# Yzmblog/SurfD

Measured on AMD Instinct MI355X. Metric: shapes/sec end-to-end (1000-step uncond, 512^3 UDF) at 1/2/4/8 GPU, higher is better.
Workload: dtype f32 (every matrix product of decoder and denoiser as three split-fp16 products on the fp16 MFMA pipe with fp32 accumulation — fp32-class error, same golden tolerances as the exact-fp32 kernels; samplers, attention, embedding MLP and grid bookkeeping in exact fp32)

## Files before the change

### surfd_amd/csrc/decoder.hip

```cpp
#include "common.h"
#include "points.h"
#include <string.h>
#include <stdlib.h>
#include <type_traits>
#include <utility>

namespace surfd {

constexpr int H = 512;
constexpr int NB = 5;
constexpr int NCBN = 2 * NB + 1;
constexpr int TP = 64;
constexpr int XS = H + 4;
constexpr int ES = 68;
constexpr int KG_H = H / 8;
constexpr int KG_E = 8;

constexpr size_t SZ_FCP = (size_t)16 * KG_E * 256;
constexpr size_t SZ_HH = (size_t)16 * KG_H * 256;
constexpr size_t SZ_FCPT = (size_t)2 * KG_H * 256;
constexpr size_t OFF_FCP = 0;
__host__ __device__ constexpr size_t off_fc(int k, int which) { return SZ_FCP + (size_t)(2 * k + which) * SZ_HH; }
__host__ __device__ constexpr size_t off_fcT(int k, int which) { return SZ_FCP + (size_t)(2 * NB + 2 * k + which) * SZ_HH; }
constexpr size_t OFF_FCPT = SZ_FCP + (size_t)4 * NB * SZ_HH;
// ... 218 lines not shown
#pragma unroll
    for (int d = REQ_EARLY ? REQ_EARLY_UPTO : WS_AHEAD; d < D - 1; ++d) load_wstage<KS>(ws.b[d], Whf, lofs, d);
#pragma unroll 1
    for (int ks0 = 0; ks0 < KS - D; ks0 += D) group(ks0, std::false_type{});
    group(KS - D, std::true_type{});
}

template <int... I, typename F>
__device__ __forceinline__ void static_for_impl(std::integer_sequence<int, I...>, F &&f) { (f(std::integral_constant<int, I>{}), ...); }
template <int N, typename F>
__device__ __forceinline__ void static_for(F &&f) { static_for_impl(std::make_integer_sequence<int, N>{}, f); }

template <int BEG, bool WITH_CHUNKS, typename ChunkFn>
__device__ __forceinline__ void gemm_half_f16x2(const float *A, const _Float16 *Whf, WStages &ws, f32x16 (&acc)[2][4], int lane, ChunkFn &&chunk) {
    constexpr int D = 4, KS = KS_H, END = BEG + 16;
    const float *a0 = A + (lane & 31) * XS + 4 * (lane >> 5);
    const float *a1 = a0 + 32 * XS;
    unsigned lofs = (unsigned)lane * 16u;
    asm volatile("" : "+v"(lofs));
    f16x8 x[2][2][2];
    auto load_x = [&](f16x8 (&dst)[2][2], int ks) {
        dst[0][0] = *reinterpret_cast<const f16x8 *>(a0 + ks * 8); dst[0][1] = *reinterpret_cast<const f16x8 *>(a0 + 256 + ks * 8);
        dst[1][0] = *reinterpret_cast<const f16x8 *>(a1 + ks * 8); dst[1][1] = *reinterpret_cast<const f16x8 *>(a1 + 256 + ks * 8);
    };
    load_x(x[0], BEG);
    if constexpr (BEG == 0) {
#pragma unroll
        for (int d = REQ_EARLY ? REQ_EARLY_UPTO : 0; d < D - 1; ++d) load_wstage<KS>(ws.b[d], Whf, lofs, d);
    }
    if constexpr (WITH_CHUNKS) {
        static_for<16>([&](auto idx) {
            constexpr int ks = BEG + decltype(idx)::value, j = ks % D;
            if constexpr (ks + D - 1 < KS) load_wstage<KS>(ws.b[(j + D - 1) % D], Whf, lofs, ks + D - 1);
            if constexpr (ks + 1 < END) load_x(x[(ks + 1) & 1], ks + 1);
            chunk(idx);
            mfma_step_f16x2(x[ks & 1], ws.b[j], acc);
#pragma unroll
            for (int i = 0; i < 8; ++i) { __builtin_amdgcn_sched_group_barrier(0x008, 1, 0); __builtin_amdgcn_sched_group_barrier(0x020, 1, 0); __builtin_amdgcn_sched_group_barrier(0x002, 1, 0); }
#pragma unroll
            for (int i = 0; i < 4; ++i) { __builtin_amdgcn_sched_group_barrier(0x008, 1, 0); __builtin_amdgcn_sched_group_barrier(0x100, 1, 0); __builtin_amdgcn_sched_group_barrier(0x002, 2, 0); }
#pragma unroll
            for (int i = 0; i < 8; ++i) { __builtin_amdgcn_sched_group_barrier(0x008, 1, 0); __builtin_amdgcn_sched_group_barrier(0x002, 2, 0); }
#pragma unroll
            for (int i = 0; i < 4; ++i) { __builtin_amdgcn_sched_group_barrier(0x008, 1, 0); __builtin_amdgcn_sched_group_barrier(0x200, 1, 0); }
            __builtin_amdgcn_sched_barrier(0);
        });
    } else {
        auto group = [&](int ks0, auto last) {
            int goff = ks0 * 8;
            asm volatile("" : "+v"(goff));
#pragma unroll
            for (int j = 0; j < D; ++j) {
                if (!decltype(last)::value || j == 0) load_wstage<KS>(ws.b[(j + D - 1) % D], Whf, lofs, ks0 + j + D - 1);
                const int jn = (decltype(last)::value && j == D - 1) ? j : j + 1;
                x[(j + 1) & 1][0][0] = *reinterpret_cast<const f16x8 *>(a0 + goff + jn * 8); x[(j + 1) & 1][0][1] = *reinterpret_cast<const f16x8 *>(a0 + goff + 256 + jn * 8);
                x[(j + 1) & 1][1][0] = *reinterpret_cast<const f16x8 *>(a1 + goff + jn * 8); x[(j + 1) & 1][1][1] = *reinterpret_cast<const f16x8 *>(a1 + goff + 256 + jn * 8);
                mfma_step_f16x2(x[j & 1], ws.b[j], acc);
#pragma unroll
                for (int i = 0; i < 8; ++i) { __builtin_amdgcn_sched_group_barrier(0x008, 1, 0); __builtin_amdgcn_sched_group_barrier(0x020, 1, 0); }
#pragma unroll
                for (int i = 0; i < 4; ++i) { __builtin_amdgcn_sched_group_barrier(0x008, 1, 0); __builtin_amdgcn_sched_group_barrier(0x100, 1, 0); }
                __builtin_amdgcn_sched_group_barrier(0x008, 12, 0);
                __builtin_amdgcn_sched_barrier(0);
            }
        };
        static_assert(END == KS, "the rolled half is the second one");
#pragma unroll 1
        for (int ks0 = BEG; ks0 < END - D; ks0 += D) group(ks0, std::false_type{});
        group(END - D, std::true_type{});
    }
}

template <int KG>
__device__ __forceinline__ void gemm_1x1(const float *A, int astride, int mt, const gfloat *Wp_tile, f32x16 &acc, int lane) {
    const float *a0 = A + (32 * mt + (lane & 31)) * astride + 4 * (lane >> 5);
    const gf32x4 *w = reinterpret_cast<const gf32x4 *>(Wp_tile) + lane;
#pragma unroll 4
    for (int kg = 0; kg < KG; ++kg) {
        const f32x4 x0 = *reinterpret_cast<const f32x4 *>(a0 + kg * 8);
        const f32x4 b = w[kg * 64];
#pragma unroll
        for (int q = 0; q < 4; ++q) acc = mfma(x0[q], b[q], acc);
    }
}

__device__ __forceinline__ void zero_acc(f32x16 (&acc)[2][4]) {
#pragma unroll
    for (int mt = 0; mt < 2; ++mt)
#pragma unroll
        for (int nt = 0; nt < 4; ++nt)
#pragma unroll
            for (int r = 0; r < 16; ++r) acc[mt][nt][r] = 0.f;
}

__device__ __forceinline__ constexpr int mword(int mt, int nt) { return (mt * 4 + nt) >> 1; }
__device__ __forceinline__ constexpr int mbit(int mt, int nt, int r) { return ((mt * 4 + nt) & 1) * 16 + r; }

template <int TPP>
__device__ __forceinline__ void encode_tile_f16x2(const PtIO &io, long e0, long npts, const float *PT, float *X, int tid, int &sat_flag) {
    constexpr int LOG2 = TPP == 8 ? 3 : 2;
    static_assert(TPP == 4 || TPP == 8, "threads per point");
    const int p = tid >> LOG2, part = tid & (TPP - 1);
    _Float16 *hrow = reinterpret_cast<_Float16 *>(reinterpret_cast<unsigned *>(X) + p * XS);
    auto put = [&](int j, float u) {
        const _Float16 h = (_Float16)u;
        hrow[j] = h;
        hrow[512 + j] = (_Float16)(u - (float)h);
    };
    if (io.mode == PT_EMB) {
        const long e = e0 + p;
        bool bad = false;
#pragma unroll 2
        for (int i = 0; i < 64 / TPP; ++i) {
            const int j = part * (64 / TPP) + i;
            float u = (e < npts && j < io.emb_dim) ? io.xyz[e * io.emb_dim + j] : 0.f;
            bad |= __builtin_fabsf(u) > 65504.f;
            u = __builtin_amdgcn_fmed3f(u, -65504.f, 65504.f);
            put(j, u);
        }
        sat_flag |= __any(bad);
        return;
    }
    const float x = PT[p * 4 + 0], y = PT[p * 4 + 1], z = PT[p * 4 + 2];
    {
        float u = part == 0 ? x : (part == 1 ? y : z);
        const bool bad = part < 3 && __builtin_fabsf(u) > 65504.f;
        sat_flag |= __any(bad);
        u = __builtin_amdgcn_fmed3f(u, -65504.f, 65504.f);
        if (part < 3) put(part, u);
        if (part == 3) put(63, 0.f);
    }
    int f = part / 3, r = part - 3 * (part / 3);
#pragma unroll
    for (int q0 = 0; q0 < 30; q0 += TPP) {
        if (q0 + part < 30) {
            const float a = (r == 0 ? x : (r == 1 ? y : z)) * (float)(1 << f);
            float sn, cs;
            sincosf(a, &sn, &cs);
            put(3 + 6 * f + r, sn);
            put(6 + 6 * f + r, cs);
        }
        r += TPP % 3; f += TPP / 3;
        if (r >= 3) { r -= 3; ++f; }
    }
}

#ifdef SURFD_DEC_STAMPS
__device__ long long g_dec_stamps[8];
#define TDECL() long long tacc_[5] = {0, 0, 0, 0, 0}, t0_ = __builtin_readcyclecounter()
#define TADD(slot) do { const long long t1_ = __builtin_readcyclecounter(); tacc_[slot] += t1_ - t0_; t0_ = t1_; } while (0)
#define TBAR() do { TADD(tphase_); __syncthreads(); TADD(3); } while (0)
#define TPHASE(x) tphase_ = (x)
#define TFLUSH() do { if (blockIdx.x == 0 && threadIdx.x == 0) { for (int i_ = 0; i_ < 5; ++i_) g_dec_stamps[i_] += tacc_[i_]; g_dec_stamps[5] += 1; } } while (0)
#else
#define TDECL()
#define TADD(slot)
#define TBAR() __syncthreads()
#define TPHASE(x)
#define TFLUSH()
#endif

template <bool GRAD, bool F16X2 = false>
__global__ __launch_bounds__(256, 1) void decoder_kernel(DecParams P, PtBatch B) {
    extern __shared__ __attribute__((aligned(16))) float lds[];
    float *X = lds;
    float *E = lds;
    float *PT = lds + TP * XS;
    float *LOG = PT + TP * 4;
    float *E2 = LOG + TP;
    float *DV = E2 + TP * ES;
    float *RED = DV + TP * 4;

    const int tid = threadIdx.x, lane = tid & 63, wave = tid >> 6;
    const int col = lane & 31;
    const int wave_u = __builtin_amdgcn_readfirstlane(wave);
    typedef float __attribute__((address_space(3))) lds_f32;
    lds_f32 *xb0 = (lds_f32 *)(X + (4 * (lane >> 5)) * XS + 128 * wave + col);
    lds_f32 *xb1 = xb0 + 32 * XS;
    auto fresh_xat_bases = [&]() { if constexpr (GRAD && F16X2) asm volatile("" : "+v"(xb0), "+v"(xb1)); };
#define XAT(mt, nt, r) ((mt) ? xb1 : xb0)[(((r) & 3) + 8 * ((r) >> 2)) * XS + 32 * (nt)]
    typedef unsigned __attribute__((address_space(3))) lds_u32;
    lds_u32 *xw0 = (lds_u32 *)(reinterpret_cast<unsigned *>(X) + (4 * (lane >> 5)) * XS + XW_WAVE * wave + col);
    lds_u32 *xw1 = xw0 + 32 * XS;
#define XW(mt, q, r, pl) ((mt) ? xw1 : xw0)[(((r) & 3) + 8 * ((r) >> 2)) * XS + XW_Q * (q) + 256 * (pl)]
    int sat_flag = 0;
    auto store_split = [&](const f32x16 (&v)[2][4], const float (&sa)[4], const float (&sb)[4], unsigned *mk, auto qn) {
        float umax = 0.f;
#pragma unroll
        for (int q = 0; q < decltype(qn)::value; ++q)
#pragma unroll
            for (int mt = 0; mt < 2; ++mt) {
                if constexpr (!GRAD && !FWD_STAGED) {
#pragma unroll
                    for (int r = 0; r < 16; ++r) {
                        const float t0 = __builtin_fmaf(sa[2 * q], v[mt][2 * q][r], sb[2 * q]);
                        const float t1 = __builtin_fmaf(sa[2 * q + 1], v[mt][2 * q + 1][r], sb[2 * q + 1]);
                        umax = __builtin_fmaxf(__builtin_fmaxf(umax, t0), t1);
                        const float u0 = __builtin_amdgcn_fmed3f(t0, 0.f, 65504.f);
                        const float u1 = __builtin_amdgcn_fmed3f(t1, 0.f, 65504.f);
                        const f32x2 u = {u0, u1};
                        const unsigned h = __builtin_bit_cast(unsigned, __builtin_convertvector(u, f16x2));
                        XW(mt, q, r, 0) = h;
                        XW(mt, q, r, 1) = split_low_pair(h, u0, u1);
                    }
                    continue;
                }
                __builtin_amdgcn_sched_barrier(0);
#pragma unroll
                for (int r0 = 0; r0 < 16; r0 += SURFD_DEC_GRAD_W) {
                    float t0[SURFD_DEC_GRAD_W], t1[SURFD_DEC_GRAD_W];
                    f32x2 u[SURFD_DEC_GRAD_W];
                    f16x2 h[SURFD_DEC_GRAD_W];
                    unsigned l[SURFD_DEC_GRAD_W];
#pragma unroll
                    for (int i = 0; i < SURFD_DEC_GRAD_W; ++i) {
                        t0[i] = __builtin_fmaf(sa[2 * q], v[mt][2 * q][r0 + i], sb[2 * q]);
                        t1[i] = __builtin_fmaf(sa[2 * q + 1], v[mt][2 * q + 1][r0 + i], sb[2 * q + 1]);
                    }
#pragma unroll
                    for (int i = 0; i < SURFD_DEC_GRAD_W; ++i) {
                        umax = __builtin_fmaxf(__builtin_fmaxf(umax, t0[i]), t1[i]);
                        if constexpr (GRAD) {
                            mk[mword(mt, 2 * q)] |= t0[i] > 0.f ? 1u << mbit(mt, 2 * q, r0 + i) : 0u;
                            mk[mword(mt, 2 * q + 1)] |= t1[i] > 0.f ? 1u << mbit(mt, 2 * q + 1, r0 + i) : 0u;
                        }
                        u[i].x = __builtin_amdgcn_fmed3f(t0[i], 0.f, 65504.f);
                        u[i].y = __builtin_amdgcn_fmed3f(t1[i], 0.f, 65504.f);
                    }
#pragma unroll
                    for (int i = 0; i < SURFD_DEC_GRAD_W; ++i) h[i] = __builtin_convertvector(u[i], f16x2);
#pragma unroll
                    for (int i = 0; i < SURFD_DEC_GRAD_W; ++i) {
#if SURFD_DEC_GRAD_MIX
                        l[i] = split_low_pair(__builtin_bit_cast(unsigned, h[i]), u[i].x, u[i].y);
#else
                        l[i] = __builtin_bit_cast(unsigned, __builtin_convertvector(u[i] - __builtin_convertvector(h[i], f32x2), f16x2));
#endif
                    }
#pragma unroll
                    for (int i = 0; i < SURFD_DEC_GRAD_W; ++i) {
                        XW(mt, q, r0 + i, 0) = __builtin_bit_cast(unsigned, h[i]);
                        XW(mt, q, r0 + i, 1) = l[i];
                    }
                }
            }
        sat_flag |= __any(umax > 65504.f);
    };
    auto split_chunk = [&](auto idx, const f32x16 (&v)[2][4], const float (&sa)[4], const float (&sb)[4], float &umax) {
#pragma unroll
        for (int i = 0; i < 2; ++i) {
            constexpr int base = 2 * decltype(idx)::value;
            const int mt = (base + i) >> 4, r = (base + i) & 15;
            const float t0 = __builtin_fmaf(sa[2], v[mt][2][r], sb[2]);
            const float t1 = __builtin_fmaf(sa[3], v[mt][3][r], sb[3]);
            umax = __builtin_fmaxf(__builtin_fmaxf(umax, t0), t1);
            const float u0 = __builtin_amdgcn_fmed3f(t0, 0.f, 65504.f);
            const float u1 = __builtin_amdgcn_fmed3f(t1, 0.f, 65504.f);
            const f32x2 u = {u0, u1};
            const f16x2 h = __builtin_convertvector(u, f16x2);
            const f32x2 hf = __builtin_convertvector(h, f32x2);
            const f32x2 rr = {u0 - hf.x, u1 - hf.y};
            const f16x2 l = __builtin_convertvector(rr, f16x2);
            XW(mt, 1, r, 0) = __builtin_bit_cast(unsigned, h);
            XW(mt, 1, r, 1) = __builtin_bit_cast(unsigned, l);
        }
    };

    WStages ws;
    if constexpr (F16X2) gemm_prefetch_f16x2<KS_E>(ws, P.whf + (size_t)(4 * wave_u) * KS_E * 2 * 512, lane);

    TDECL(); int tphase_ = 0; (void)tphase_;
    for (int bi = 0; bi < B.n; ++bi) {
    const PtIO &io = B.io[bi];
    const long npts = pt_count(io);
    const long ntiles = (npts + TP - 1) / TP;
    const float *tab_sample = P.tab + (size_t)B.sample[bi] * NCBN * 2 * H;
    const long tstep = io.shard_n > 1 ? io.shard_n : 1;
    for (long tile = blockIdx.x * tstep + (io.shard_n > 1 ? io.shard_i : 0); tile < ntiles; tile += gridDim.x * tstep) {
        const long e0 = tile * TP;
        const float *wpack_ = P.wpack, *vecs_ = P.vecs, *tab_ = tab_sample;
        const _Float16 *whf = P.whf;
        int tid_tile = threadIdx.x;
        if constexpr (GRAD && F16X2) asm volatile("" : "+v"(tid_tile));
        const int tid = tid_tile, lane = tid & 63, wave = tid >> 6, col = lane & 31;
        int cb = 128 * wave + col;
        asm volatile("" : "+s"(wpack_), "+s"(vecs_), "+s"(tab_));
        if constexpr (F16X2) asm volatile("" : "+s"(whf), "+v"(cb), "+v"(xw0), "+v"(xw1));
        const gfloat *wpack = (const gfloat *)wpack_, *vecs = (const gfloat *)vecs_, *tab = (const gfloat *)tab_;
        TPHASE(4);
        TBAR();
        if (tid < TP) {
            const long e = e0 + tid;
            float x = 0.f, y = 0.f, z = 0.f;
            int vox = -1;
            if (e < npts) {
                if (io.mode == PT_XYZ) {
                    x = io.xyz[e * 3 + 0]; y = io.xyz[e * 3 + 1]; z = io.xyz[e * 3 + 2];
                    vox = 0;
                } else if (io.mode == PT_EMB) {
                    vox = 0;
                } else {
                    vox = pt_voxel(io, e);
                    voxel_xyz(io, vox, x, y, z);
                }
            }
            PT[tid * 4 + 0] = x; PT[tid * 4 + 1] = y; PT[tid * 4 + 2] = z;
            PT[tid * 4 + 3] = __int_as_float(vox);
// ... 368 lines not shown
            } else {
#pragma unroll
            for (int k = NB - 1; k >= 0; --k) {
#pragma unroll
                for (int mt = 0; mt < 2; ++mt)
#pragma unroll
                    for (int nt = 0; nt < 4; ++nt)
#pragma unroll
                        for (int r = 0; r < 16; ++r)
                            XAT(mt, nt, r) = g[mt][nt][r];
                __syncthreads();
                zero_acc(tmp);
                gemm_2x4<KG_H>(X, XS, wpack + off_fcT(k, 1) + (size_t)(4 * wave) * KG_H * 256, tmp, lane);
                __syncthreads();
                {
                    float sa[4];
#pragma unroll
                    for (int nt = 0; nt < 4; ++nt) sa[nt] = tab[(2 * k + 1) * 2 * H + 32 * (4 * wave + nt) + col];
#pragma unroll
                    for (int mt = 0; mt < 2; ++mt)
#pragma unroll
                        for (int nt = 0; nt < 4; ++nt)
#pragma unroll
                            for (int r = 0; r < 16; ++r) {
                                const bool on = (msk[2 * k + 1][mword(mt, nt)] >> mbit(mt, nt, r)) & 1u;
                                XAT(mt, nt, r) = on ? tmp[mt][nt][r] * sa[nt] : 0.f;
                            }
                }
                __syncthreads();
                zero_acc(tmp);
                gemm_2x4<KG_H>(X, XS, wpack + off_fcT(k, 0) + (size_t)(4 * wave) * KG_H * 256, tmp, lane);
                {
                    float sa[4];
#pragma unroll
                    for (int nt = 0; nt < 4; ++nt) sa[nt] = tab[(2 * k) * 2 * H + 32 * (4 * wave + nt) + col];
#pragma unroll
                    for (int mt = 0; mt < 2; ++mt)
#pragma unroll
                        for (int nt = 0; nt < 4; ++nt)
#pragma unroll
                            for (int r = 0; r < 16; ++r) {
                                const bool on = (msk[2 * k][mword(mt, nt)] >> mbit(mt, nt, r)) & 1u;
                                g[mt][nt][r] += on ? tmp[mt][nt][r] * sa[nt] : 0.f;
                            }
                }
                __syncthreads();
            }
            }
            fresh_xat_bases();
#pragma unroll
            for (int mt = 0; mt < 2; ++mt)
#pragma unroll
                for (int nt = 0; nt < 4; ++nt)
#pragma unroll
                    for (int r = 0; r < 16; ++r)
                        XAT(mt, nt, r) = g[mt][nt][r];
            __syncthreads();
            {
                f32x16 ea;
#pragma unroll
                for (int r = 0; r < 16; ++r) ea[r] = 0.f;
                const int mt = wave & 1, et = wave >> 1;
                gemm_1x1<KG_H>(X, XS, mt, wpack + OFF_FCPT + (size_t)et * KG_H * 256, ea, lane);
#pragma unroll
                for (int r = 0; r < 16; ++r) E2[(32 * mt + frag_row(r, lane)) * ES + 32 * et + col] = ea[r];
            }
            __syncthreads();
            if (tid < TP * 3) {
                const int p = tid / 3, c = tid % 3;
                const float xc = PT[p * 4 + c];
                float d = E2[p * ES + c];
#pragma unroll
                for (int j = 0; j < 10; ++j) {
                    const float f = (float)(1 << j);
                    float sn, cs;
                    sincosf(xc * f, &sn, &cs);
                    d += f * (cs * E2[p * ES + 3 + 6 * j + c] - sn * E2[p * ES + 6 + 6 * j + c]);
                }
                DV[p * 4 + c] = d;
            }
            __syncthreads();
            if (tid < TP) {
                const long e = e0 + tid;
                if (e < npts) {
                    const float o = LOG[tid];
                    const float y = 1.f / (1.f + expf(-o));
                    const float udf = (1.f - y) * 0.1f;
                    const float sfac = -0.1f * ((1.f - y) * y);
                    const float gx = sfac * DV[tid * 4 + 0], gy = sfac * DV[tid * 4 + 1], gz = sfac * DV[tid * 4 + 2];
                    const float nrm = fmaxf(sqrtf(gx * gx + gy * gy + gz * gz), 1e-12f);
                    const float ox = -(gx / nrm), oy = -(gy / nrm), oz = -(gz / nrm);
                    if (io.out_logit) io.out_logit[e] = o;
                    if (io.out_udf) io.out_udf[e] = udf;
                    if (io.out_dlogit) { io.out_dlogit[e * 3 + 0] = DV[tid * 4 + 0]; io.out_dlogit[e * 3 + 1] = DV[tid * 4 + 1]; io.out_dlogit[e * 3 + 2] = DV[tid * 4 + 2]; }
                    if (io.out_ngrad) { io.out_ngrad[e * 3 + 0] = ox; io.out_ngrad[e * 3 + 1] = oy; io.out_ngrad[e * 3 + 2] = oz; }
                    if (io.grid_grads) {
                        const long vox = __float_as_int(PT[tid * 4 + 3]);
                        io.grid_grads[vox * 3 + 0] = ox; io.grid_grads[vox * 3 + 1] = oy; io.grid_grads[vox * 3 + 2] = oz;
                    }
                }
            }
        }
    }
    }
    if constexpr (F16X2) {
        if (sat_flag && lane == 0) atomicAdd(P.sat, 1u);
    }
    TFLUSH();
}

#undef XAT

struct WStages8 { f16x8 b[4][2][2]; };

template <int KS>
__device__ __forceinline__ void load_wstage8(f16x8 (&dst)[2][2], const _Float16 *Whf, unsigned lofs, int ks) {
    const unsigned long long wa = (unsigned long long)Whf;
    unsigned wlo = __builtin_amdgcn_readfirstlane((unsigned)wa), whi = __builtin_amdgcn_readfirstlane((unsigned)(wa >> 32));
    asm volatile("" : "+s"(wlo), "+s"(whi));
    const __attribute__((address_space(1))) char *wb = (const __attribute__((address_space(1))) char *)(((unsigned long long)whi << 32) | wlo);
#pragma unroll
    for (int nt = 0; nt < 2; ++nt)
#pragma unroll
        for (int q = 0; q < 2; ++q)
#if defined(SURFD_DEC_W_NT) && SURFD_DEC_W_NT
            dst[nt][q] = __builtin_nontemporal_load(reinterpret_cast<const gf16x8 *>(wb + (size_t)(nt * KS * 2048) + (lofs + (unsigned)((ks * 2 + q) * 1024))));
#else
            dst[nt][q] = *reinterpret_cast<const gf16x8 *>(wb + (size_t)(nt * KS * 2048) + (lofs + (unsigned)((ks * 2 + q) * 1024)));
#endif
}

__device__ __forceinline__ void mfma_step8(const f16x8 (&a)[2][2], const f16x8 (&b)[2][2], f32x16 (&acc)[2][2]) {
    constexpr int TA[3] = {1, 0, 0};
    constexpr int TB[3] = {0, 1, 0};
#pragma unroll
    for (int t = 0; t < 3; ++t)
#pragma unroll
        for (int nt = 0; nt < 2; ++nt)
#pragma unroll
            for (int mt = 0; mt < 2; ++mt)
                acc[mt][nt] = __builtin_amdgcn_mfma_f32_32x32x16_f16(a[mt][TA[t]], b[nt][TB[t]], acc[mt][nt], 0, 0, 0);
}

template <int KS>
__device__ __forceinline__ void gemm8_request(WStages8 &ws, const _Float16 *Whf, int lane) {
    __builtin_amdgcn_sched_barrier(0);
    unsigned lofs = (unsigned)lane * 16u;
    asm volatile("" : "+v"(lofs));
    load_wstage8<KS>(ws.b[0], Whf, lofs, 0);
    __builtin_amdgcn_sched_barrier(0);
}

template <int KS>
__device__ __forceinline__ void gemm8(const float *A, const _Float16 *Whf, WStages8 &ws, f32x16 (&acc)[2][2], int lane) {
    constexpr int D = 4;
    static_assert(KS % D == 0, "k-step count must be a multiple of the pipeline depth");
    const float *a0 = A + (lane & 31) * XS + 4 * (lane >> 5);
    const float *a1 = a0 + 32 * XS;
    unsigned lofs = (unsigned)lane * 16u;
    asm volatile("" : "+v"(lofs));
    f16x8 x[2][2][2];
    auto group = [&](int ks0, auto last) {
        int goff = ks0 * 8;
        asm volatile("" : "+v"(goff));
#pragma unroll
        for (int j = 0; j < D; ++j) {
            if (!decltype(last)::value || j == 0) load_wstage8<KS>(ws.b[(j + D - 1) % D], Whf, lofs, ks0 + j + D - 1);
            const int jn = (decltype(last)::value && j == D - 1) ? j : j + 1;
            x[(j + 1) & 1][0][0] = *reinterpret_cast<const f16x8 *>(a0 + goff + jn * 8); x[(j + 1) & 1][0][1] = *reinterpret_cast<const f16x8 *>(a0 + goff + 256 + jn * 8);
            x[(j + 1) & 1][1][0] = *reinterpret_cast<const f16x8 *>(a1 + goff + jn * 8); x[(j + 1) & 1][1][1] = *reinterpret_cast<const f16x8 *>(a1 + goff + 256 + jn * 8);
            mfma_step8(x[j & 1], ws.b[j], acc);
#pragma unroll
            for (int i = 0; i < 4; ++i) { __builtin_amdgcn_sched_group_barrier(0x008, 1, 0); __builtin_amdgcn_sched_group_barrier(0x020, 1, 0); }
#pragma unroll
            for (int i = 0; i < 4; ++i) { __builtin_amdgcn_sched_group_barrier(0x008, 1, 0); __builtin_amdgcn_sched_group_barrier(0x100, 1, 0); }
            __builtin_amdgcn_sched_group_barrier(0x008, 4, 0);
            __builtin_amdgcn_sched_barrier(0);
        }
    };
    x[0][0][0] = *reinterpret_cast<const f16x8 *>(a0); x[0][0][1] = *reinterpret_cast<const f16x8 *>(a0 + 256);
    x[0][1][0] = *reinterpret_cast<const f16x8 *>(a1); x[0][1][1] = *reinterpret_cast<const f16x8 *>(a1 + 256);
    if constexpr (KS > D) {
#pragma unroll
        for (int d = 1; d < D - 1; ++d) load_wstage8<KS>(ws.b[d], Whf, lofs, d);
#pragma unroll 1
        for (int ks0 = 0; ks0 < KS - D; ks0 += D) group(ks0, std::false_type{});
        group(KS - D, std::true_type{});
    } else {
#pragma unroll
        for (int d = 1; d < D; ++d) load_wstage8<KS>(ws.b[d], Whf, lofs, d);
        int goff = 0;
        asm volatile("" : "+v"(goff));
#pragma unroll
        for (int j = 0; j < D; ++j) {
            const int jn = j == D - 1 ? j : j + 1;
            x[(j + 1) & 1][0][0] = *reinterpret_cast<const f16x8 *>(a0 + goff + jn * 8); x[(j + 1) & 1][0][1] = *reinterpret_cast<const f16x8 *>(a0 + goff + 256 + jn * 8);
            x[(j + 1) & 1][1][0] = *reinterpret_cast<const f16x8 *>(a1 + goff + jn * 8); x[(j + 1) & 1][1][1] = *reinterpret_cast<const f16x8 *>(a1 + goff + 256 + jn * 8);
            mfma_step8(x[j & 1], ws.b[j], acc);
            __builtin_amdgcn_sched_barrier(0);
        }
    }
}

__global__ __launch_bounds__(512, 1) void decoder_fwd8_kernel(DecParams P, PtBatch B) {
    extern __shared__ __attribute__((aligned(16))) float lds[];
    float *X = lds;
    float *PT = lds + TP * XS;
    float *LOG = PT + TP * 4;
    const int tid = threadIdx.x, lane = tid & 63, wave = tid >> 6;
    const int col = lane & 31;
    const int wave_u = __builtin_amdgcn_readfirstlane(wave);
    float *const xb0 = X + (4 * (lane >> 5)) * XS + 64 * wave + col;
    float *const xb1 = xb0 + 32 * XS;
#define XAT8(mt, nt, r) ((mt) ? xb1 : xb0)[(((r) & 3) + 8 * ((r) >> 2)) * XS + 32 * (nt)]
    typedef unsigned __attribute__((address_space(3))) lds_u32;
    lds_u32 *xw0 = (lds_u32 *)(reinterpret_cast<unsigned *>(X) + (4 * (lane >> 5)) * XS + 32 * wave + col);
    lds_u32 *xw1 = xw0 + 32 * XS;
#define XW8(mt, r, pl) ((mt) ? xw1 : xw0)[(((r) & 3) + 8 * ((r) >> 2)) * XS + 256 * (pl)]
#ifndef SURFD_DEC_XCD_STAGGER
#define SURFD_DEC_XCD_STAGGER 0
#endif
#if SURFD_DEC_XCD_STAGGER > 0
    for (int k_ = 0; k_ < (int)(blockIdx.x & 7) * SURFD_DEC_XCD_STAGGER; ++k_) __builtin_amdgcn_s_sleep(127);
#endif
#ifndef SURFD_DEC_CLOCK
#define SURFD_DEC_CLOCK 1
#endif
#if SURFD_DEC_CLOCK
    unsigned long long *const clk = reinterpret_cast<unsigned long long *>(P.sat + 2);
    unsigned long long *const clk0 = reinterpret_cast<unsigned long long *>(LOG + TP);
    if (blockIdx.x == 0 && tid == 0) {
        clk0[0] = (unsigned long long)__builtin_readcyclecounter();
        clk0[1] = (unsigned long long)__builtin_amdgcn_s_memrealtime();
    }
#endif
    int sat_flag = 0;
    auto store8 = [&](const f32x16 (&v)[2][2], const float (&sa)[2], const float (&sb)[2]) {
        float umax = 0.f;
#pragma unroll
        for (int mt = 0; mt < 2; ++mt)
#pragma unroll
            for (int r = 0; r < 16; ++r) {
                const float t0 = __builtin_fmaf(sa[0], v[mt][0][r], sb[0]);
                const float t1 = __builtin_fmaf(sa[1], v[mt][1][r], sb[1]);
                umax = __builtin_fmaxf(__builtin_fmaxf(umax, t0), t1);
                const float u0 = __builtin_amdgcn_fmed3f(t0, 0.f, 65504.f);
                const float u1 = __builtin_amdgcn_fmed3f(t1, 0.f, 65504.f);
                const f32x2 u = {u0, u1};
                const unsigned h = __builtin_bit_cast(unsigned, __builtin_convertvector(u, f16x2));
                XW8(mt, r, 0) = h;
                XW8(mt, r, 1) = split_low_pair(h, u0, u1);
            }
        sat_flag |= __any(umax > 65504.f);
    };
    auto zero8 = [](f32x16 (&a)[2][2]) {
#pragma unroll
        for (int mt = 0; mt < 2; ++mt)
#pragma unroll
            for (int nt = 0; nt < 2; ++nt)
#pragma unroll
                for (int r = 0; r < 16; ++r) a[mt][nt][r] = 0.f;
    };
    WStages8 ws;
    for (int bi = 0; bi < B.n; ++bi) {
    const PtIO &io = B.io[bi];
    const long npts = pt_count(io);
    const long ntiles = (npts + TP - 1) / TP;
    const float *tab_sample = P.tab + (size_t)B.sample[bi] * NCBN * 2 * H;
    const long tstep = io.shard_n > 1 ? io.shard_n : 1;
    for (long tile = blockIdx.x * tstep + (io.shard_n > 1 ? io.shard_i : 0); tile < ntiles; tile += gridDim.x * tstep) {
        const long e0 = tile * TP;
        const float *vecs_ = P.vecs, *tab_ = tab_sample;
        const _Float16 *whf = P.whf;
        unsigned cb = 64 * wave + col;
        asm volatile("" : "+s"(vecs_), "+s"(tab_), "+s"(whf), "+v"(cb), "+v"(xw0), "+v"(xw1));
        const gfloat *vecs = (const gfloat *)vecs_, *tab = (const gfloat *)tab_;
        const size_t woff_e = (size_t)(2 * wave_u) * KS_E * 2 * 512, woff = (size_t)(2 * wave_u) * KS_H * 2 * 512;
        __syncthreads();
        {
        int tid_fe = threadIdx.x;
        asm volatile("" : "+v"(tid_fe));
        const int tid = tid_fe;
        if (tid < TP) {
            const long e = e0 + tid;
            float x = 0.f, y = 0.f, z = 0.f;
            int vox = -1;
            if (e < npts) {
                if (io.mode == PT_XYZ) { x = io.xyz[e * 3 + 0]; y = io.xyz[e * 3 + 1]; z = io.xyz[e * 3 + 2]; vox = 0; }
                else if (io.mode == PT_EMB) vox = 0;
                else { vox = pt_voxel(io, e); voxel_xyz(io, vox, x, y, z); }
            }
            PT[tid * 4 + 0] = x; PT[tid * 4 + 1] = y; PT[tid * 4 + 2] = z;
            PT[tid * 4 + 3] = __int_as_float(vox);
        }
        __syncthreads();
        encode_tile_f16x2<8>(io, e0, npts, PT, X, tid, sat_flag);
        }
        gemm8_request<KS_E>(ws, whf + woff_e, lane);
        __syncthreads();
        f32x16 net[2][2], tmp[2][2];
        zero8(net);
        const float winv = vecs[VOFF_SC + 1];
        float nsa[2], nsb[2];
#pragma unroll
        for (int nt = 0; nt < 2; ++nt) {
            const unsigned c = cb + 32 * nt;
            const float a = tab[c];
            nsa[nt] = a * winv;
            nsb[nt] = __builtin_fmaf(a, vecs[voff_cb(0) + c], tab[H + c]);
        }
        gemm8<KS_E>(X, whf + woff_e, ws, net, lane);
        __syncthreads();
#pragma unroll 1
        for (int k = 0; k < NB; ++k) {
            const _Float16 *W0 = whf + (HF_FCP + (size_t)(2 * k) * HF_HH) + woff, *W1 = W0 + HF_HH;
            {
                float sa[2] = {nsa[0], nsa[1]}, sb[2] = {nsb[0], nsb[1]};
                store8(net, sa, sb);
            }
            gemm8_request<KS_H>(ws, W0, lane);
            __syncthreads();
            zero8(tmp);
            float sa1[2], sbb[2];
#pragma unroll
            for (int nt = 0; nt < 2; ++nt) {
                const unsigned c = cb + 32 * nt;
                const float a = tab[(2 * k + 1) * 2 * H + c];
                sa1[nt] = a * winv;
                sbb[nt] = __builtin_fmaf(a, vecs[H * (1 + 2 * k) + c], tab[(2 * k + 1) * 2 * H + H + c]);
            }
            gemm8<KS_H>(X, W0, ws, tmp, lane);
            __syncthreads();
            store8(tmp, sa1, sbb);
            gemm8_request<KS_H>(ws, W1, lane);
            __syncthreads();
#pragma unroll
            for (int nt = 0; nt < 2; ++nt) {
                const unsigned c = cb + 32 * nt;
                const float a = tab[(2 * k + 2) * 2 * H + c];
                nsa[nt] = a * winv;
                nsb[nt] = __builtin_fmaf(a, vecs[voff_cb(0) + H * (k + 1) + c], tab[(2 * k + 2) * 2 * H + H + c]);
            }
            gemm8<KS_H>(X, W1, ws, net, lane);
            __syncthreads();
        }
        {
#pragma unroll
            for (int nt = 0; nt < 2; ++nt) {
                const float wo = vecs[VOFF_WOUT + cb + 32 * nt];
#pragma unroll
                for (int mt = 0; mt < 2; ++mt)
#pragma unroll
                    for (int r = 0; r < 16; ++r) {
                        const float u = nsa[nt] * net[mt][nt][r] + nsb[nt];
                        XAT8(mt, nt, r) = fmaxf(u, 0.f) * wo;
                    }
            }
        }
        __syncthreads();
        {
            const float bo = vecs[VOFF_BOUT];
            for (int pp = 0; pp < TP / 8; ++pp) {
                const int p = wave * (TP / 8) + pp;
                float sacc = 0.f;
#pragma unroll
                for (int i = 0; i < H / 64; ++i) sacc += X[p * XS + lane + 64 * i];
#pragma unroll
                for (int off = 32; off > 0; off >>= 1) sacc += __shfl_xor(sacc, off);
                if (lane == 0) LOG[p] = sacc + bo;
            }
        }
        __syncthreads();
        if (tid < TP) {
            const long e = e0 + tid;
            const bool valid = e < npts;
            float udf = 0.f;
            int vox = 0;
            if (valid) {
                const float o = LOG[tid];
                const float y = 1.f / (1.f + expf(-o));
                udf = (1.f - y) * 0.1f;
                if (io.out_logit) io.out_logit[e] = o;
                if (io.out_udf) io.out_udf[e] = udf;
                if (io.grid_udf) {
                    vox = __float_as_int(PT[tid * 4 + 3]);
                    io.grid_udf[vox] = udf;
                }
            }
            if (io.grid_udf && io.grad_list) {
                const int slot = wave_append_slot(io.grad_count, valid && udf < io.grad_thr);
                if (slot >= 0) io.grad_list[slot] = vox;
            }
        }
    }
    }
    if (sat_flag && lane == 0) atomicAdd(P.sat, 1u);
#if SURFD_DEC_CLOCK
    if (blockIdx.x == 0 && tid == 0) {
        const unsigned long long c1 = (unsigned long long)__builtin_readcyclecounter(), r1 = (unsigned long long)__builtin_amdgcn_s_memrealtime();
        atomicAdd(clk + 2, c1 - clk0[0]);
        atomicAdd(clk + 3, r1 - clk0[1]);
    }
#endif
}
#undef XAT8
#undef XW8

#undef XW
constexpr size_t DEC_LDS_BYTES = (size_t)(TP * XS + TP * 4 + TP + TP * ES + TP * 4 + 4) * sizeof(float);

__global__ void absmax_kernel(const float *src, size_t n, unsigned *out) {
    unsigned m = 0u;
    for (size_t i = blockIdx.x * (size_t)blockDim.x + threadIdx.x; i < n; i += (size_t)gridDim.x * blockDim.x)
        m = max(m, __float_as_uint(src[i]) & 0x7fffffffu);
#pragma unroll
    for (int off = 32; off > 0; off >>= 1) m = max(m, (unsigned)__shfl_xor((int)m, off));
    if ((threadIdx.x & 63) == 0 && m) atomicMax(out, m);
}

__global__ void weight_scale_kernel(const unsigned *maxbits, float *sc) {
    const unsigned b = *maxbits;
    int e = (int)(b >> 23) - 127;
    if (b == 0u || e > 100 || e < -100) e = 8;
    sc[0] = __uint_as_float((unsigned)(127 + 8 - e) << 23);
    sc[1] = __uint_as_float((unsigned)(127 - 8 + e) << 23);
}

__global__ void pack_f16x2_kernel(const float *wp, int KG, int KS, int permute, const float *sc, _Float16 *dst) {
    const float scale = sc[0];
    const long total = (long)16 * KS * 64 * 8;
    for (long e = blockIdx.x * (long)blockDim.x + threadIdx.x; e < total; e += (long)gridDim.x * blockDim.x) {
        const int el = e & 7, lane = (e >> 3) & 63;
        const long tk = e >> 9;
        const int ks = tk % KS, tile = tk / KS;
        const int slot = ks * 16 + 8 * (lane >> 5) + el;
        const int k = permute ? slot_channel(slot) : slot;
        const float x = wp[((size_t)(tile * KG + (k >> 3)) * 64 + (lane & 31) + 32 * ((k >> 2) & 1)) * 4 + (k & 3)] * scale;
        const _Float16 h = (_Float16)x;
        const _Float16 l = (_Float16)(x - (float)h);
        const size_t base = ((size_t)(tile * KS + ks) * 2) * 512 + (size_t)lane * 8 + el;
        dst[base] = h; dst[base + 512] = l;
    }
}

__global__ void cumbias_kernel(float *vecs) {
    const int c = blockIdx.x * blockDim.x + threadIdx.x;
    if (c >= H) return;
    float acc = vecs[VOFF_BFCP + c];
    vecs[voff_cb(0) + c] = acc;
    for (int k = 0; k < NB; ++k) { acc += vecs[voff_bfc(k, 1) + c]; vecs[voff_cb(k + 1) + c] = acc; }
}

struct CbnParams {
    const float *gw[NCBN], *gb[NCBN], *bw[NCBN], *bb[NCBN], *mean[NCBN], *var[NCBN];
};

__global__ void cbn_table_kernel(CbnParams P, const float *lat, int S, int D, float *tab) {
    const int total = S * NCBN * H;
    for (int e = blockIdx.x * blockDim.x + threadIdx.x; e < total; e += gridDim.x * blockDim.x) {
        const int c = e % H, l = (e / H) % NCBN, s = e / (H * NCBN);
        float gamma = 0.f, beta = 0.f;
        for (int d = 0; d < D; ++d) {
            const float z = lat[s * D + d];
            gamma += P.gw[l][c * D + d] * z;
            beta += P.bw[l][c * D + d] * z;
        }
        gamma += P.gb[l][c];
        beta += P.bb[l][c];
        const float a = gamma / sqrtf(P.var[l][c] + 1e-5f);
        tab[((size_t)(s * NCBN + l) * 2 + 0) * H + c] = a;
        tab[((size_t)(s * NCBN + l) * 2 + 1) * H + c] = beta - a * P.mean[l][c];
    }
}

}

#define DEC_STR_(x) #x
#define DEC_STR(x) DEC_STR_(x)
#if defined(SURFD_DEC_W_NT) && SURFD_DEC_W_NT
#define DEC_CFG_W_NT 1
#else
#define DEC_CFG_W_NT 0
#endif
#if defined(SURFD_DEC_STAMPS)
#define DEC_CFG_STAMPS 1
#else
#define DEC_CFG_STAMPS 0
#endif
#if SURFD_DEC_OVL != 0 && !defined(SURFD_ALLOW_UNSAFE_VARIANTS)
#error "SURFD_DEC_OVL=1 is an experiment kept as a record (profiles/r03_decoder_variants.md); -DSURFD_ALLOW_UNSAFE_VARIANTS builds it anyway"
#endif
namespace surfd {
const char *decoder_build_config() {
    return "DEC_OVL=" DEC_STR(SURFD_DEC_OVL) " DEC_MIX=" DEC_STR(SURFD_DEC_MIX) " DEC_GRAD_W=" DEC_STR(SURFD_DEC_GRAD_W) " DEC_GRAD_MIX=" DEC_STR(SURFD_DEC_GRAD_MIX)
           " DEC_WS_AHEAD=" DEC_STR(SURFD_DEC_WS_AHEAD) " DEC_REQ_EARLY=" DEC_STR(SURFD_DEC_REQ_EARLY) " DEC_FWD_STAGED=" DEC_STR(SURFD_DEC_FWD_STAGED)
           " DEC_XCD_STAGGER=" DEC_STR(SURFD_DEC_XCD_STAGGER) " DEC_CLOCK=" DEC_STR(SURFD_DEC_CLOCK) " DEC_W_NT=" DEC_STR(DEC_CFG_W_NT) " DEC_STAMPS=" DEC_STR(DEC_CFG_STAMPS);
}
int decoder_build_unsafe() { return SURFD_DEC_OVL != 0; }
}

using namespace surfd;

struct DecTensor {
    std::string key;
    std::vector<int64_t> shape;
    bool is_set = false;
};

struct surfd_decoder {
    int input_dim = 63, D = 32, hidden = 512, nb = 5, device = -1;
    std::vector<DecTensor> params;
    std::map<std::string, int> index;
    bool allocated = false, finalized = false;
    float *wpack = nullptr, *vecs = nullptr;
    _Float16 *whf = nullptr;
    int precision = 1;
    int fwd8 = 1;
    float *gw[NCBN] = {}, *gb[NCBN] = {}, *bw[NCBN] = {}, *bb[NCBN] = {}, *mean[NCBN] = {}, *var[NCBN] = {};
    float *tab = nullptr;
    int S = 0, tab_cap = 0;
    int num_cus = 256;
    int grid_blocks = 0;
    unsigned *sat = nullptr;
    std::vector<void *> allocs;
};

static void dec_add(surfd_decoder *d, const std::string &k, std::vector<int64_t> shape) {
    d->index[k] = (int)d->params.size();
    d->params.push_back({k, std::move(shape)});
}

static void dec_add_cbn(surfd_decoder *d, const std::string &p) {
    const int64_t Hh = d->hidden, D = d->D;
    dec_add(d, p + ".conv_gamma.weight", {Hh, D, 1}); dec_add(d, p + ".conv_gamma.bias", {Hh});
    dec_add(d, p + ".conv_beta.weight", {Hh, D, 1});  dec_add(d, p + ".conv_beta.bias", {Hh});
    dec_add(d, p + ".bn.running_mean", {Hh});         dec_add(d, p + ".bn.running_var", {Hh});
    dec_add(d, p + ".bn.num_batches_tracked", {});
}

static int dec_alloc(surfd_decoder *d) {
    if (d->allocated) return SURFD_OK;
    HIP_TRY(hipGetDevice(&d->device));
    hipDeviceProp_t prop;
    HIP_TRY(hipGetDeviceProperties(&prop, d->device));
    d->num_cus = prop.multiProcessorCount;
    auto A = [&](float **p, size_t n) -> int {
        HIP_TRY(hipMalloc((void **)p, n * sizeof(float)));
        d->allocs.push_back(*p);
// ... 332 lines not shown
```

Baseline: 4.913.

## Overlap next-tile point fetch and encoding with decoder hidden-layer GEMMs

Restructures the persistent fwd8 decoder loop into a software pipeline. The next tile's point coordinates and voxel indices are prefetched during the embedding GEMM, and its positional encoding is built in four slices into a separate LDS region interleaved with the residual blocks. The first-layer weights are also prefetched before the tile ends, and the final logit reduction and output write are merged into one step, which removes two barriers. The aim is to hide encode and gather latency and cut synchronisation, at the cost of more LDS, extra registers, and more complex control flow, with a risk of lower occupancy or scheduling regressions.

```diff
diff --git a/surfd_amd/csrc/decoder.hip b/surfd_amd/csrc/decoder.hip
--- a/surfd_amd/csrc/decoder.hip
+++ b/surfd_amd/csrc/decoder.hip
@@ -394,7 +394,17 @@
 #define TBAR() do { TADD(tphase_); __syncthreads(); TADD(3); } while (0)
 #define TPHASE(x) tphase_ = (x)
 #define TFLUSH() do { if (blockIdx.x == 0 && threadIdx.x == 0) { for (int i_ = 0; i_ < 5; ++i_) g_dec_stamps[i_] += tacc_[i_]; g_dec_stamps[5] += 1; } } while (0)
+#define T8DECL() unsigned t8acc_[7] = {0, 0, 0, 0, 0, 0, 0}, t8n_ = 0, t8_0_ = (unsigned)__builtin_readcyclecounter()
+#define T8ADD(slot) do { const unsigned t1_ = (unsigned)__builtin_readcyclecounter(); t8acc_[slot] += t1_ - t8_0_; t8_0_ = t1_; } while (0)
+#define T8BAR(slot) do { T8ADD(slot); __syncthreads(); T8ADD(5); } while (0)
+#define T8TILE() (++t8n_)
+#define T8FLUSH() do { if (blockIdx.x == 0 && threadIdx.x == 0) { for (int i_ = 0; i_ < 7; ++i_) g_dec_stamps[i_] += t8acc_[i_]; g_dec_stamps[7] += t8n_; } } while (0)
 #else
+#define T8DECL()
+#define T8ADD(slot)
+#define T8BAR(slot) __syncthreads()
+#define T8TILE()
+#define T8FLUSH()
 #define TDECL()
 #define TADD(slot)
 #define TBAR() __syncthreads()
@@ -1069,11 +1079,22 @@
 }
 
 template <int KS>
+__device__ __forceinline__ void gemm8_request_all(WStages8 &ws, const _Float16 *Whf, int lane) {
+    static_assert(KS == 4, "one stage per k-step");
+    __builtin_amdgcn_sched_barrier(0);
+    unsigned lofs = (unsigned)lane * 16u;
+    asm volatile("" : "+v"(lofs));
+#pragma unroll
+    for (int d = 0; d < 4; ++d) load_wstage8<KS>(ws.b[d], Whf, lofs, d);
+    __builtin_amdgcn_sched_barrier(0);
+}
+
+template <int KS, int AS = XS, int APL = 256>
 __device__ __forceinline__ void gemm8(const float *A, const _Float16 *Whf, WStages8 &ws, f32x16 (&acc)[2][2], int lane) {
     constexpr int D = 4;
     static_assert(KS % D == 0, "k-step count must be a multiple of the pipeline depth");
-    const float *a0 = A + (lane & 31) * XS + 4 * (lane >> 5);
-    const float *a1 = a0 + 32 * XS;
+    const float *a0 = A + (lane & 31) * AS + 4 * (lane >> 5);
+    const float *a1 = a0 + 32 * AS;
     unsigned lofs = (unsigned)lane * 16u;
     asm volatile("" : "+v"(lofs));
     f16x8 x[2][2][2];
@@ -1084,8 +1105,8 @@
         for (int j = 0; j < D; ++j) {
             if (!decltype(last)::value || j == 0) load_wstage8<KS>(ws.b[(j + D - 1) % D], Whf, lofs, ks0 + j + D - 1);
             const int jn = (decltype(last)::value && j == D - 1) ? j : j + 1;
-            x[(j + 1) & 1][0][0] = *reinterpret_cast<const f16x8 *>(a0 + goff + jn * 8); x[(j + 1) & 1][0][1] = *reinterpret_cast<const f16x8 *>(a0 + goff + 256 + jn * 8);
-            x[(j + 1) & 1][1][0] = *reinterpret_cast<const f16x8 *>(a1 + goff + jn * 8); x[(j + 1) & 1][1][1] = *reinterpret_cast<const f16x8 *>(a1 + goff + 256 + jn * 8);
+            x[(j + 1) & 1][0][0] = *reinterpret_cast<const f16x8 *>(a0 + goff + jn * 8); x[(j + 1) & 1][0][1] = *reinterpret_cast<const f16x8 *>(a0 + goff + APL + jn * 8);
+            x[(j + 1) & 1][1][0] = *reinterpret_cast<const f16x8 *>(a1 + goff + jn * 8); x[(j + 1) & 1][1][1] = *reinterpret_cast<const f16x8 *>(a1 + goff + APL + jn * 8);
             mfma_step8(x[j & 1], ws.b[j], acc);
 #pragma unroll
             for (int i = 0; i < 4; ++i) { __builtin_amdgcn_sched_group_barrier(0x008, 1, 0); __builtin_amdgcn_sched_group_barrier(0x020, 1, 0); }
@@ -1095,8 +1116,8 @@
             __builtin_amdgcn_sched_barrier(0);
         }
     };
-    x[0][0][0] = *reinterpret_cast<const f16x8 *>(a0); x[0][0][1] = *reinterpret_cast<const f16x8 *>(a0 + 256);
-    x[0][1][0] = *reinterpret_cast<const f16x8 *>(a1); x[0][1][1] = *reinterpret_cast<const f16x8 *>(a1 + 256);
+    x[0][0][0] = *reinterpret_cast<const f16x8 *>(a0); x[0][0][1] = *reinterpret_cast<const f16x8 *>(a0 + APL);
+    x[0][1][0] = *reinterpret_cast<const f16x8 *>(a1); x[0][1][1] = *reinterpret_cast<const f16x8 *>(a1 + APL);
     if constexpr (KS > D) {
 #pragma unroll
         for (int d = 1; d < D - 1; ++d) load_wstage8<KS>(ws.b[d], Whf, lofs, d);
@@ -1104,18 +1125,83 @@
         for (int ks0 = 0; ks0 < KS - D; ks0 += D) group(ks0, std::false_type{});
         group(KS - D, std::true_type{});
     } else {
-#pragma unroll
-        for (int d = 1; d < D; ++d) load_wstage8<KS>(ws.b[d], Whf, lofs, d);
         int goff = 0;
         asm volatile("" : "+v"(goff));
 #pragma unroll
         for (int j = 0; j < D; ++j) {
             const int jn = j == D - 1 ? j : j + 1;
-            x[(j + 1) & 1][0][0] = *reinterpret_cast<const f16x8 *>(a0 + goff + jn * 8); x[(j + 1) & 1][0][1] = *reinterpret_cast<const f16x8 *>(a0 + goff + 256 + jn * 8);
-            x[(j + 1) & 1][1][0] = *reinterpret_cast<const f16x8 *>(a1 + goff + jn * 8); x[(j + 1) & 1][1][1] = *reinterpret_cast<const f16x8 *>(a1 + goff + 256 + jn * 8);
+            x[(j + 1) & 1][0][0] = *reinterpret_cast<const f16x8 *>(a0 + goff + jn * 8); x[(j + 1) & 1][0][1] = *reinterpret_cast<const f16x8 *>(a0 + goff + APL + jn * 8);
+            x[(j + 1) & 1][1][0] = *reinterpret_cast<const f16x8 *>(a1 + goff + jn * 8); x[(j + 1) & 1][1][1] = *reinterpret_cast<const f16x8 *>(a1 + goff + APL + jn * 8);
             mfma_step8(x[j & 1], ws.b[j], acc);
             __builtin_amdgcn_sched_barrier(0);
         }
+    }
+}
+
+__device__ __forceinline__ int pt_voxel_raw(const PtIO &io, long e) {
+    const unsigned ee = (unsigned)e;
+    switch (io.mode) {
+        case PT_LIST: return io.list[e];
+        case PT_CHILDREN: return io.list[ee / 7u];
+        case PT_CHILDREN8: return io.list[ee >> 3];
+        default: return 0;
+    }
+}
+__device__ __forceinline__ int pt_voxel_from_raw(const PtIO &io, long e, int raw) {
+    const unsigned ee = (unsigned)e;
+    switch (io.mode) {
+        case PT_LIST: return raw;
+        case PT_CHILDREN: {
+            const int c = (int)(ee - 7u * (ee / 7u)) + 1;
+            return raw + (((c >> 2) & 1) * io.N * io.N + ((c >> 1) & 1) * io.N + (c & 1)) * io.s;
+        }
+        case PT_CHILDREN8: {
+            const int c = (int)(ee & 7u);
+            return raw + (((c >> 2) & 1) * io.N * io.N + ((c >> 1) & 1) * io.N + (c & 1)) * io.s;
+        }
+        default: return pt_voxel(io, e);
+    }
+}
+
+__device__ __forceinline__ void encode_slice8(const PtIO &io, long e0, long npts, const float *PT, float *EN, int tid, int &sat_flag, int sl) {
+    const int p = tid >> 3, part = tid & 7;
+    _Float16 *hrow = reinterpret_cast<_Float16 *>(reinterpret_cast<unsigned *>(EN) + p * ES);
+    auto put = [&](int j, float u) {
+        const _Float16 h = (_Float16)u;
+        hrow[j] = h;
+        hrow[64 + j] = (_Float16)(u - (float)h);
+    };
+    if (io.mode == PT_EMB) {
+        if (sl != 0) return;
+        const long e = e0 + p;
+        bool bad = false;
+#pragma unroll 2
+        for (int i = 0; i < 8; ++i) {
+            const int j = part * 8 + i;
+            float u = (e < npts && j < io.emb_dim) ? io.xyz[e * io.emb_dim + j] : 0.f;
+            bad |= __builtin_fabsf(u) > 65504.f;
+            u = __builtin_amdgcn_fmed3f(u, -65504.f, 65504.f);
+            put(j, u);
+        }
+        sat_flag |= __any(bad);
+        return;
+    }
+    if (sl == 0) {
+        float u = part < 3 ? PT[p * 4 + part] : 0.f;
+        const bool bad = part < 3 && __builtin_fabsf(u) > 65504.f;
+        sat_flag |= __any(bad);
+        u = __builtin_amdgcn_fmed3f(u, -65504.f, 65504.f);
+        if (part < 3) put(part, u);
+        if (part == 3) put(63, 0.f);
+    }
+    const int q = 8 * sl + part;
+    if (q < 30) {
+        const int f = q / 3, r = q - 3 * f;
+        const float a = PT[p * 4 + r] * (float)(1 << f);
+        float sn, cs;
+        sincosf(a, &sn, &cs);
+        put(3 + 6 * f + r, sn);
+        put(6 + 6 * f + r, cs);
     }
 }
 
@@ -1124,6 +1210,8 @@
     float *X = lds;
     float *PT = lds + TP * XS;
     float *LOG = PT + TP * 4;
+    float *EN = LOG + TP;
+    float *CLK0 = EN + TP * ES + TP * 4;
     const int tid = threadIdx.x, lane = tid & 63, wave = tid >> 6;
     const int col = lane & 31;
     const int wave_u = __builtin_amdgcn_readfirstlane(wave);
@@ -1145,13 +1233,14 @@
 #endif
 #if SURFD_DEC_CLOCK
     unsigned long long *const clk = reinterpret_cast<unsigned long long *>(P.sat + 2);
-    unsigned long long *const clk0 = reinterpret_cast<unsigned long long *>(LOG + TP);
+    unsigned long long *const clk0 = reinterpret_cast<unsigned long long *>(CLK0);
     if (blockIdx.x == 0 && tid == 0) {
         clk0[0] = (unsigned long long)__builtin_readcyclecounter();
         clk0[1] = (unsigned long long)__builtin_amdgcn_s_memrealtime();
     }
 #endif
     int sat_flag = 0;
+    T8DECL();
     auto store8 = [&](const f32x16 (&v)[2][2], const float (&sa)[2], const float (&sb)[2]) {
         float umax = 0.f;
 #pragma unroll
@@ -1185,19 +1274,15 @@
     const long ntiles = (npts + TP - 1) / TP;
     const float *tab_sample = P.tab + (size_t)B.sample[bi] * NCBN * 2 * H;
     const long tstep = io.shard_n > 1 ? io.shard_n : 1;
-    for (long tile = blockIdx.x * tstep + (io.shard_n > 1 ? io.shard_i : 0); tile < ntiles; tile += gridDim.x * tstep) {
-        const long e0 = tile * TP;
-        const float *vecs_ = P.vecs, *tab_ = tab_sample;
-        const _Float16 *whf = P.whf;
-        unsigned cb = 64 * wave + col;
-        asm volatile("" : "+s"(vecs_), "+s"(tab_), "+s"(whf), "+v"(cb), "+v"(xw0), "+v"(xw1));
-        const gfloat *vecs = (const gfloat *)vecs_, *tab = (const gfloat *)tab_;
-        const size_t woff_e = (size_t)(2 * wave_u) * KS_E * 2 * 512, woff = (size_t)(2 * wave_u) * KS_H * 2 * 512;
-        __syncthreads();
-        {
+    const long tstride = gridDim.x * tstep;
+    long tile = blockIdx.x * tstep + (io.shard_n > 1 ? io.shard_i : 0);
+    if (tile >= ntiles) continue;
+    {
+        T8BAR(6);
         int tid_fe = threadIdx.x;
         asm volatile("" : "+v"(tid_fe));
         const int tid = tid_fe;
+        const long e0 = tile * TP;
         if (tid < TP) {
             const long e = e0 + tid;
             float x = 0.f, y = 0.f, z = 0.f;
@@ -1210,11 +1295,33 @@
             PT[tid * 4 + 0] = x; PT[tid * 4 + 1] = y; PT[tid * 4 + 2] = z;
             PT[tid * 4 + 3] = __int_as_float(vox);
         }
-        __syncthreads();
-        encode_tile_f16x2<8>(io, e0, npts, PT, X, tid, sat_flag);
-        }
-        gemm8_request<KS_E>(ws, whf + woff_e, lane);
-        __syncthreads();
+        T8BAR(0);
+#pragma unroll 1
+        for (int sl = 0; sl < 4; ++sl) encode_slice8(io, e0, npts, PT, EN, tid, sat_flag, sl);
+        gemm8_request_all<KS_E>(ws, P.whf + (size_t)(2 * wave_u) * KS_E * 2 * 512, lane);
+        T8BAR(1);
+    }
+    for (; tile < ntiles; tile += tstride) {
+        const long e0 = tile * TP;
+        const bool have_next = tile + tstride < ntiles;
+        const long e0n = e0 + tstride * TP;
+        const float *vecs_ = P.vecs, *tab_ = tab_sample;
+        const _Float16 *whf = P.whf;
+        unsigned cb = 64 * wave + col;
+        asm volatile("" : "+s"(vecs_), "+s"(tab_), "+s"(whf), "+v"(cb), "+v"(xw0), "+v"(xw1));
+        const gfloat *vecs = (const gfloat *)vecs_, *tab = (const gfloat *)tab_;
+        const size_t woff_e = (size_t)(2 * wave_u) * KS_E * 2 * 512, woff = (size_t)(2 * wave_u) * KS_H * 2 * 512;
+        float fx = 0.f, fy = 0.f, fz = 0.f;
+        int fraw = 0;
+        if (have_next && wave_u == 0) {
+            const long e = e0n + lane;
+            if (e < npts) {
+                if (io.mode == PT_XYZ) { fx = io.xyz[e * 3 + 0]; fy = io.xyz[e * 3 + 1]; fz = io.xyz[e * 3 + 2]; }
+                else if (io.mode != PT_EMB) fraw = pt_voxel_raw(io, e);
+            }
+        }
+        __builtin_amdgcn_sched_barrier(0);
+        T8ADD(0);
         f32x16 net[2][2], tmp[2][2];
         zero8(net);
         const float winv = vecs[VOFF_SC + 1];
@@ -1226,8 +1333,24 @@
             nsa[nt] = a * winv;
             nsb[nt] = __builtin_fmaf(a, vecs[voff_cb(0) + c], tab[H + c]);
         }
-        gemm8<KS_E>(X, whf + woff_e, ws, net, lane);
-        __syncthreads();
+        gemm8<KS_E, ES, 32>(EN, whf + woff_e, ws, net, lane);
+        T8BAR(2);
+        if (wave_u == 0) {
+            int lane_fe = threadIdx.x;
+            asm volatile("" : "+v"(lane_fe));
+            LOG[lane_fe] = PT[lane_fe * 4 + 3];
+            if (have_next) {
+                const long e = e0n + lane_fe;
+                int vox = -1;
+                if (e < npts) {
+                    if (io.mode == PT_XYZ || io.mode == PT_EMB) vox = 0;
+                    else { vox = pt_voxel_from_raw(io, e, fraw); voxel_xyz(io, vox, fx, fy, fz); }
+                }
+                PT[lane_fe * 4 + 0] = fx; PT[lane_fe * 4 + 1] = fy; PT[lane_fe * 4 + 2] = fz;
+                PT[lane_fe * 4 + 3] = __int_as_float(vox);
+            }
+        }
+        T8ADD(0);
 #pragma unroll 1
         for (int k = 0; k < NB; ++k) {
             const _Float16 *W0 = whf + (HF_FCP + (size_t)(2 * k) * HF_HH) + woff, *W1 = W0 + HF_HH;
@@ -1236,7 +1359,7 @@
                 store8(net, sa, sb);
             }
             gemm8_request<KS_H>(ws, W0, lane);
-            __syncthreads();
+            T8BAR(4);
             zero8(tmp);
             float sa1[2], sbb[2];
 #pragma unroll
@@ -1247,10 +1370,16 @@
                 sbb[nt] = __builtin_fmaf(a, vecs[H * (1 + 2 * k) + c], tab[(2 * k + 1) * 2 * H + H + c]);
             }
             gemm8<KS_H>(X, W0, ws, tmp, lane);
-            __syncthreads();
+            T8BAR(3);
             store8(tmp, sa1, sbb);
             gemm8_request<KS_H>(ws, W1, lane);
-            __syncthreads();
+            T8ADD(4);
+            if (have_next && k < 4) {
+                int tid_fe = threadIdx.x;
+                asm volatile("" : "+v"(tid_fe));
+                encode_slice8(io, e0n, npts, PT, EN, tid_fe, sat_flag, k);
+            }
+            T8BAR(1);
 #pragma unroll
             for (int nt = 0; nt < 2; ++nt) {
                 const unsigned c = cb + 32 * nt;
@@ -1259,8 +1388,9 @@
                 nsb[nt] = __builtin_fmaf(a, vecs[voff_cb(0) + H * (k + 1) + c], tab[(2 * k + 2) * 2 * H + H + c]);
             }
             gemm8<KS_H>(X, W1, ws, net, lane);
-            __syncthreads();
-        }
+            T8BAR(3);
+        }
+        if (have_next) gemm8_request_all<KS_E>(ws, whf + woff_e, lane);
         {
 #pragma unroll
             for (int nt = 0; nt < 2; ++nt) {
@@ -1274,33 +1404,34 @@
                     }
             }
         }
-        __syncthreads();
+        T8BAR(6);
         {
+            int tid_fe = threadIdx.x;
+            asm volatile("" : "+v"(tid_fe));
+            const int lane = tid_fe & 63, p0 = (tid_fe >> 6) * (TP / 8);
             const float bo = vecs[VOFF_BOUT];
+            float o = 0.f;
+#pragma unroll
             for (int pp = 0; pp < TP / 8; ++pp) {
-                const int p = wave * (TP / 8) + pp;
                 float sacc = 0.f;
 #pragma unroll
-                for (int i = 0; i < H / 64; ++i) sacc += X[p * XS + lane + 64 * i];
+                for (int i = 0; i < H / 64; ++i) sacc += X[(p0 + pp) * XS + lane + 64 * i];
 #pragma unroll
                 for (int off = 32; off > 0; off >>= 1) sacc += __shfl_xor(sacc, off);
-                if (lane == 0) LOG[p] = sacc + bo;
-            }
-        }
-        __syncthreads();
-        if (tid < TP) {
-            const long e = e0 + tid;
-            const bool valid = e < npts;
+                if (lane == pp) o = sacc + bo;
+            }
+            const int p = p0 + (lane & 7);
+            const long e = e0 + p;
+            const bool valid = lane < TP / 8 && e < npts;
             float udf = 0.f;
             int vox = 0;
             if (valid) {
-                const float o = LOG[tid];
                 const float y = 1.f / (1.f + expf(-o));
                 udf = (1.f - y) * 0.1f;
                 if (io.out_logit) io.out_logit[e] = o;
                 if (io.out_udf) io.out_udf[e] = udf;
                 if (io.grid_udf) {
-                    vox = __float_as_int(PT[tid * 4 + 3]);
+                    vox = __float_as_int(LOG[p]);
                     io.grid_udf[vox] = udf;
                 }
             }
@@ -1309,8 +1440,12 @@
                 if (slot >= 0) io.grad_list[slot] = vox;
             }
         }
-    }
-    }
+        T8ADD(6);
+        T8TILE();
+    }
+    }
+    T8ADD(6);
+    T8FLUSH();
     if (sat_flag && lane == 0) atomicAdd(P.sat, 1u);
 #if SURFD_DEC_CLOCK
     if (blockIdx.x == 0 && tid == 0) {
```

Result: no change. 4.914 (median of 3 runs) (+0.0%).
